# cielavenir/7bgzf

Measured on AMD Instinct MI355X. Metric: GB/s input compressed, BGZF 64KiB blocks, higher is better.
Workload: dtype u8

## Files before the change

7bgzf_amd/__init__.py:

```python
import ctypes
import os

import numpy as np

HERE = os.path.dirname(os.path.abspath(__file__))
LIB_PATH = os.path.join(HERE, "libhipdeflate.so")

FRAME_RAW, FRAME_BGZF, FRAME_MIGZ, FRAME_RAW_FLUSH, FRAME_ZLIB, FRAME_GZIP = 0, 1, 2, 3, 4, 5
FRAME_LATENCY = 0x100
DEFLATE_HIP = 11
HD_E_NODEVICE, HD_E_ARG, HD_E_NOMEM = 100, 101, 102

BGZF_BLOCK = 0xff00
WG_LEVEL = 3
BGZF_EOF = bytes.fromhex("1f8b08040000000000ff0600424302001b0003000000000000000000")


class HipDeflateError(RuntimeError):
    pass


_lib = None
_vp = ctypes.c_void_p


class MemberSummary(ctypes.Structure):
    _fields_ = [("nmembers", ctypes.c_uint64), ("out_bytes", ctypes.c_uint64), ("end_offset", ctypes.c_uint64),
                ("status", ctypes.c_uint32)]


class RangeSummary(ctypes.Structure):
    _fields_ = [("out_bytes", ctypes.c_uint64), ("nselected", ctypes.c_uint64), ("sel_bytes", ctypes.c_uint64),
                ("nrefused", ctypes.c_uint64), ("bad_member", ctypes.c_uint64), ("status", ctypes.c_uint32)]


class StreamSummary(ctypes.Structure):
    _fields_ = [("out_bytes", ctypes.c_uint64), ("in_bytes", ctypes.c_uint64), ("bad_chunk", ctypes.c_uint64),
                ("nchunks", ctypes.c_uint32), ("check", ctypes.c_uint32), ("status", ctypes.c_uint32)]


class StreamIndexSummary(ctypes.Structure):
    _fields_ = [("nchunks", ctypes.c_uint64), ("out_bytes", ctypes.c_uint64), ("end_offset", ctypes.c_uint64),
                ("ncandidates", ctypes.c_uint64), ("hdr_bytes", ctypes.c_uint32), ("status", ctypes.c_uint32)]


STREAM_WINDOW_BYTES = 1 << 30
CHECK_CRC32, CHECK_ADLER32 = 0, 1
RANGE_BYTES, RANGE_VOFFSET = 0, 1
RANGE_PIECE = 256 << 10


def voffset(coffset, uoffset):
    return (int(coffset) << 16) | (int(uoffset) & 0xffff)


EXPORTS = [
    "hipdeflate_init", "hipdeflate_shutdown", "hipdeflate_available", "hipdeflate_version", "hipdeflate_stall_count",
    "hip_deflate", "hip_deflate_flush", "hip_inflate", "hipdeflate_batch_deflate", "hipdeflate_batch_inflate",
    "hipdeflate_batch_deflate_dev", "hipdeflate_batch_inflate_dev", "hipdeflate_scan_sizes_dev",
    "hipdeflate_compact_dev", "hipdeflate_scratch_bytes", "bgzf_compress", "hipdeflate_selftest",
    "hipdeflate_pipe_open", "hipdeflate_pipe_input", "hipdeflate_pipe_submit", "hipdeflate_pipe_result",
    "hipdeflate_pipe_close", "hipdeflate_unpipe_open", "hipdeflate_unpipe_input", "hipdeflate_unpipe_submit",
    "hipdeflate_unpipe_result", "hipdeflate_unpipe_close", "hipdeflate_test_build_lengths", "hipdeflate_test_beside",
    "hip_inflate_flush", "hipdeflate_batch_inflate_flush", "hipdeflate_batch_inflate_flush_dev", "hipdeflate_bound",
    "hipdeflate_compact_span_dev", "hipdeflate_index_members_dev", "hipdeflate_verify_members_dev",
    "hipdeflate_read_ranges_dev",
    "hipdeflate_stream_bound", "hipdeflate_stream_deflate_dev", "hipdeflate_stream_inflate_dev",
    "hipdeflate_check_combine_dev", "hip_deflate_stream", "hipdeflate_test_stream_window",
    "hipdeflate_stream_index_dev", "hipdeflate_stream_inflate_table_dev", "hip_inflate_stream",
    "hipdeflate_init_devices", "hipdeflate_device_count", "hipdeflate_use_device",
    "hipdeflate_pipe_open_on", "hipdeflate_unpipe_open_on", "hipdeflate_lat_open_on",
    "hipdeflate_batch_inflate_size_dev", "hipdeflate_batch_inflate_framed_dev", "hipdeflate_batch_inflate_size",
    "hipdeflate_batch_inflate_framed",
    "hipdeflate_pipe_members", "hipdeflate_lat_open", "hipdeflate_lat_input", "hipdeflate_lat_run", "hipdeflate_lat_output", "hipdeflate_lat_close",
]


def _link_hip_runtime():
    import importlib.util
    spec = importlib.util.find_spec("torch")
    link = os.path.join(HERE, "hiprt", "libamdhip64.so.7")
    target = None
    if spec is not None and spec.submodule_search_locations:
        cand = os.path.join(list(spec.submodule_search_locations)[0], "lib", "libamdhip64.so")
        if os.path.exists(cand):
            target = cand
    try:
        if target is None:
            if os.path.islink(link) or os.path.exists(link):
                os.remove(link)
        elif not (os.path.islink(link) and os.readlink(link) == target):
            os.makedirs(os.path.dirname(link), exist_ok=True)
            if os.path.islink(link) or os.path.exists(link):
                os.remove(link)
            os.symlink(target, link)
    except OSError:
        pass


def lib():
    global _lib
    if _lib is not None:
        return _lib
    if not os.path.exists(LIB_PATH):
        raise HipDeflateError(
            "%s is missing: build it with `python -c 'import __graft_entry__ as g; g.build()'` "
            "(make -C 7bgzf_amd/csrc). There is no CPU fallback." % LIB_PATH)
    _link_hip_runtime()
    L = ctypes.CDLL(LIB_PATH)
    L.hipdeflate_version.restype = ctypes.c_char_p
    L.hipdeflate_scratch_bytes.restype = ctypes.c_uint64
    L.hipdeflate_bound.restype = ctypes.c_uint64
    L.hipdeflate_bound.argtypes = [ctypes.c_uint64, ctypes.c_int]
    L.hipdeflate_init.argtypes = [ctypes.c_int]
    L.hipdeflate_stall_count.restype = ctypes.c_uint64
    L.hipdeflate_stall_count.argtypes = []
    L.hipdeflate_init_devices.argtypes = [_vp, ctypes.c_int]
    L.hipdeflate_use_device.argtypes = [ctypes.c_int]
    L.hipdeflate_pipe_open_on.restype = _vp
    L.hipdeflate_pipe_open_on.argtypes = [ctypes.c_int, ctypes.c_int, ctypes.c_int, ctypes.c_uint32, ctypes.c_uint32, ctypes.c_int]
    L.hipdeflate_unpipe_open_on.restype = _vp
    L.hipdeflate_unpipe_open_on.argtypes = [ctypes.c_int, ctypes.c_uint32, ctypes.c_size_t, ctypes.c_size_t, ctypes.c_int]
    L.hipdeflate_lat_open_on.restype = _vp
    L.hipdeflate_lat_open_on.argtypes = [ctypes.c_int, ctypes.c_int, ctypes.c_int, ctypes.c_uint32, ctypes.c_uint32]
    sz_p = ctypes.POINTER(ctypes.c_size_t)
    L.hip_deflate.argtypes = [_vp, sz_p, _vp, ctypes.c_size_t, ctypes.c_int]
# ... 16 lines not shown
    L.hipdeflate_batch_inflate_framed.argtypes = [_vp, _vp, _vp, ctypes.c_uint32, ctypes.c_int, _vp, _vp, _vp, _vp, _vp, _vp, _vp]
    L.hipdeflate_scan_sizes_dev.argtypes = [_vp, ctypes.c_uint32, ctypes.c_uint64, _vp, _vp, _vp]
    L.hipdeflate_compact_dev.argtypes = [_vp, ctypes.c_uint64, _vp, _vp, ctypes.c_uint32, _vp, _vp]
    L.hipdeflate_compact_span_dev.argtypes = [_vp, ctypes.c_uint64, _vp, _vp, ctypes.c_uint32, _vp, ctypes.c_uint64, _vp]
    L.hipdeflate_index_members_dev.argtypes = [_vp, ctypes.c_uint64, ctypes.c_uint32, _vp, _vp, _vp, _vp, _vp,
                                               ctypes.POINTER(MemberSummary), _vp]
    L.hipdeflate_verify_members_dev.argtypes = [_vp, _vp, _vp, _vp, _vp, ctypes.c_uint32, ctypes.POINTER(ctypes.c_uint64), _vp]
    L.hipdeflate_read_ranges_dev.argtypes = [_vp, _vp, _vp, _vp, _vp, _vp, ctypes.c_uint32, ctypes.c_int, _vp, _vp, ctypes.c_uint32,
                                             _vp, ctypes.c_uint64, _vp, _vp, _vp, ctypes.POINTER(RangeSummary), _vp]
    L.hipdeflate_stream_bound.restype = ctypes.c_uint64
    L.hipdeflate_stream_bound.argtypes = [ctypes.c_uint64, ctypes.c_uint32, ctypes.c_int, ctypes.c_int]
    L.hipdeflate_stream_deflate_dev.argtypes = [_vp, ctypes.c_uint64, ctypes.c_uint32, ctypes.c_int, ctypes.c_int, _vp,
                                                ctypes.c_uint64, _vp, ctypes.POINTER(StreamSummary), _vp]
    L.hipdeflate_stream_inflate_dev.argtypes = [_vp, ctypes.c_uint64, ctypes.c_int, _vp, ctypes.c_uint32, ctypes.c_uint32,
                                                ctypes.c_uint64, _vp, ctypes.c_uint64, ctypes.POINTER(StreamSummary), _vp]
    L.hipdeflate_check_combine_dev.argtypes = [_vp, _vp, ctypes.c_uint32, ctypes.c_int, ctypes.POINTER(ctypes.c_uint32), _vp]
    L.hip_deflate_stream.argtypes = [_vp, sz_p, _vp, ctypes.c_size_t, ctypes.c_int, ctypes.c_int, ctypes.c_uint32]
    L.hipdeflate_stream_index_dev.argtypes = [_vp, ctypes.c_uint64, ctypes.c_int, ctypes.c_uint32, ctypes.c_uint32, _vp, _vp, _vp, _vp,
                                              ctypes.POINTER(StreamIndexSummary), _vp]
    L.hipdeflate_stream_inflate_table_dev.argtypes = [_vp, ctypes.c_uint64, ctypes.c_int, _vp, _vp, _vp, _vp, ctypes.c_uint32, _vp,
                                                      ctypes.c_uint64, ctypes.POINTER(StreamSummary), _vp]
    L.hip_inflate_stream.argtypes = [_vp, sz_p, _vp, ctypes.c_size_t, ctypes.c_int, sz_p]
    L.hipdeflate_test_stream_window.argtypes = [ctypes.c_uint32]
    L.hipdeflate_test_stream_window.restype = None
    L.hipdeflate_pipe_open.restype = _vp
    L.hipdeflate_pipe_open.argtypes = [ctypes.c_int, ctypes.c_int, ctypes.c_uint32, ctypes.c_uint32, ctypes.c_int]
    L.hipdeflate_pipe_input.restype = _vp
    L.hipdeflate_pipe_input.argtypes = [_vp, sz_p]
    L.hipdeflate_pipe_submit.argtypes = [_vp, ctypes.c_size_t]
    L.hipdeflate_pipe_result.argtypes = [_vp, ctypes.POINTER(_vp), sz_p, ctypes.POINTER(ctypes.c_uint32)]
    L.hipdeflate_pipe_members.argtypes = [_vp, ctypes.POINTER(_vp), ctypes.POINTER(_vp), ctypes.POINTER(_vp)]
    L.hipdeflate_pipe_close.restype = None
    L.hipdeflate_pipe_close.argtypes = [_vp]
    L.hipdeflate_unpipe_open.restype = _vp
    L.hipdeflate_unpipe_open.argtypes = [ctypes.c_uint32, ctypes.c_size_t, ctypes.c_size_t, ctypes.c_int]
    L.hipdeflate_unpipe_input.restype = _vp
    L.hipdeflate_unpipe_input.argtypes = [_vp, sz_p]
    L.hipdeflate_unpipe_submit.argtypes = [_vp, _vp, _vp, _vp, ctypes.c_uint32]
    L.hipdeflate_unpipe_result.argtypes = [_vp, ctypes.POINTER(_vp), sz_p]
    L.hipdeflate_unpipe_close.restype = None
    L.hipdeflate_unpipe_close.argtypes = [_vp]
    L.hipdeflate_lat_open.restype = _vp
    L.hipdeflate_lat_open.argtypes = [ctypes.c_int, ctypes.c_int, ctypes.c_uint32, ctypes.c_uint32]
    L.hipdeflate_lat_input.restype = _vp
    L.hipdeflate_lat_input.argtypes = [_vp, ctypes.c_uint32]
    L.hipdeflate_lat_run.argtypes = [_vp, _vp, ctypes.c_uint32]
    L.hipdeflate_lat_output.restype = _vp
    L.hipdeflate_lat_output.argtypes = [_vp, ctypes.c_uint32, _vp, _vp, _vp]
    L.hipdeflate_lat_close.restype = None
    L.hipdeflate_lat_close.argtypes = [_vp]
    L.hipdeflate_test_build_lengths.argtypes = [_vp, ctypes.c_uint32, ctypes.c_uint32, ctypes.c_uint32, _vp]
    L.hipdeflate_test_beside.argtypes = [ctypes.c_int, ctypes.c_uint32]
    L.hipdeflate_test_beside.restype = None
    _lib = L
    return L


def _check(rc, what):
    if rc:
        raise HipDeflateError("%s failed with %d%s" % (
            what, rc, " (no usable gfx950 device; there is no CPU fallback)" if rc == HD_E_NODEVICE else ""))


def available():
    return lib().hipdeflate_available() == 0


def version():
    lib().hipdeflate_available()
    return lib().hipdeflate_version().decode()


def _np(a, dtype):
    return np.ascontiguousarray(a, dtype=dtype)


def _p(a):
    return a.ctypes.data_as(_vp)


def as_u8(data):
    if isinstance(data, np.ndarray):
        return np.ascontiguousarray(data, dtype=np.uint8)
    return np.frombuffer(bytes(data), dtype=np.uint8) if len(data) else np.zeros(0, dtype=np.uint8)




def hip_deflate(data, level=1, cap=None):
    src = as_u8(data)
    cap = (len(src) + len(src) // 2 + 64) if cap is None else cap
    dst = np.zeros(max(cap, 1), dtype=np.uint8)
    n = ctypes.c_size_t(cap)
    r = lib().hip_deflate(_p(dst), ctypes.byref(n), _p(src), len(src), level)
    return r, bytes(dst[: n.value]) if r == 0 else b""


def hip_deflate_flush(data, level=1, cap=None):
    src = as_u8(data)
    cap = (len(src) + len(src) // 2 + 64) if cap is None else cap
    dst = np.zeros(max(cap, 1), dtype=np.uint8)
    n = ctypes.c_size_t(cap)
    r = lib().hip_deflate_flush(_p(dst), ctypes.byref(n), _p(src), len(src), level)
    return r, bytes(dst[: n.value]) if r == 0 else b""


# ... 258 lines not shown
```

7bgzf_amd/csrc/hd_api.hip:

```cpp
#include <hip/hip_runtime.h>
#include <stdio.h>
#include <stdlib.h>
#include <string.h>
#include <chrono>
#include <condition_variable>
#include <mutex>
#include <vector>

#include "../../include/hipdeflate.h"
#include "hd_call_batch.h"
#include "hd_deflate_static.hpp"
#include "hd_deflate_dynamic.hpp"
#include "hd_deflate_wg.hpp"
#include "hd_emit_wg.hpp"
#include "hd_inflate.hpp"
#include "hd_inflate_lat.hpp"
#include "hd_inflate_size.hpp"
#include "hd_frame.hpp"
#include "hd_compact.hpp"
#include "hd_index.hpp"
#include "hd_range.hpp"
#include "hd_stream.hpp"
#include "hd_segment.hpp"
#include "hd_tables.hpp"
// ... 54 lines not shown
			return 0;
		void *old = p;
		const size_t old_cap = cap;
		p = nullptr;
		cap = 0;
		const int r = reserve(n);
		if (r) {
			p = old;
			cap = old_cap;
			return r;
		}
		if (old)
			retired.push_back(old);
		return r;
	}
};

struct SharedScratch {
	Buf buf;
	hipEvent_t ev = nullptr;
	hipStream_t last = nullptr;
	bool used = false;
	int enter(hipStream_t st)
	{
		if (!ev)
			HD_CHECK(hipEventCreateWithFlags(&ev, hipEventDisableTiming));
		if (used && last != st)
			HD_CHECK(hipStreamWaitEvent(st, ev, 0));
		return 0;
	}
	int leave(hipStream_t st)
	{
		HD_CHECK(hipEventRecord(ev, st));
		last = st;
		used = true;
		return 0;
	}
	void drained(hipStream_t st)
	{
		if (last == st)
			used = false;
	}
	void reset()
	{
		buf.release();
		if (ev)
			(void)hipEventDestroy(ev);
		ev = nullptr;
		last = nullptr;
		used = false;
	}
};

struct Ctx {
	bool ready = false;
	int failed = 0;
	int device = -1;
	char desc[256] = "hipdeflate (not initialised)";
	hipStream_t stream = nullptr;
	CrcTables *d_ct = nullptr;
	uint32_t *d_stalls = nullptr;
	std::mutex mu;
	Buf d_in, d_meta, d_slots, d_packed, d_scratch;
	Buf h_in{ nullptr, 0, true }, h_meta{ nullptr, 0, true }, h_out{ nullptr, 0, true };
	std::mutex mu_dev;
	SharedScratch tok, tiles;
	SharedScratch frame;
	hd::WgBeside beside;
	void stream_drained(hipStream_t st)
	{
		std::lock_guard<std::mutex> lk(mu_dev);
		tok.drained(st);
		tiles.drained(st);
		frame.drained(st);
	}
	std::mutex mu_index;
	Buf d_index, d_cand;
	Buf d_range, d_range_out;
	Buf d_stream, d_stream_slots;
};

constexpr int HD_MAX_CTX = 32;
Ctx g_all[HD_MAX_CTX];
int g_want[HD_MAX_CTX];
int g_nctx = 0;
thread_local int t_cur = 0;
std::mutex g_init_mu;
inline Ctx &cur() { return g_all[t_cur]; }

}
int hd_probe_lds_order(void);
namespace {
constexpr int CODEC_LEVELS = 13;
constexpr size_t CODEC_POOL_MAX = 64;
std::mutex g_codec_mu;
std::vector<hipdeflate_lat *> g_codec_free[CODEC_LEVELS];
void codec_pool_drain()
{
	std::lock_guard<std::mutex> lk(g_codec_mu);
	for (std::vector<hipdeflate_lat *> &f : g_codec_free) {
		for (hipdeflate_lat *c : f)
			hipdeflate_lat_close(c);
		f.clear();
	}
}

void build_crc_tables(CrcTables *t)
{
	const uint32_t poly = 0xEDB88320u;
	for (uint32_t i = 0; i < 256; i++) {
		uint32_t c = i;
		for (int k = 0; k < 8; k++)
			c = (c >> 1) ^ (poly & (0u - (c & 1u)));
		t->T[0][i] = c;
	}
	for (int k = 1; k < 4; k++)
		for (uint32_t i = 0; i < 256; i++)
			t->T[k][i] = (t->T[k - 1][i] >> 8) ^ t->T[0][t->T[k - 1][i] & 0xff];
	for (int k = 0; k < 4; k++)
		for (uint32_t i = 0; i < 256; i++) {
			uint32_t s = i << (8 * k);
// ... 390 lines not shown

int hipdeflate_use_device(int index)
{
	if (index < 0 || index >= hipdeflate_device_count())
		return HD_E_ARG;
	t_cur = index;
	return ensure();
}

int hipdeflate_available(void) { return ensure(); }

uint64_t hipdeflate_stall_count(void)
{
	uint64_t sum = 0;
	std::lock_guard<std::mutex> lk(g_init_mu);
	for (int i = 0; i < HD_MAX_CTX; i++) {
		Ctx &g = g_all[i];
		if (!g.ready || !g.d_stalls)
			continue;
		uint32_t v = 0;
		if (hipSetDevice(g.device) == hipSuccess && hipDeviceSynchronize() == hipSuccess &&
		    hipMemcpy(&v, g.d_stalls, 4, hipMemcpyDeviceToHost) == hipSuccess)
			sum += v;
	}
	return sum;
}

const char *hipdeflate_version(void) { return cur().desc; }

static void infb_drain();

void hipdeflate_shutdown(void)
{
	codec_pool_drain();
	infb_drain();
	std::lock_guard<std::mutex> lk(g_init_mu);
	for (int i = 0; i < HD_MAX_CTX; i++) {
		Ctx &g = g_all[i];
		g.failed = 0;
		if (!g.ready)
			continue;
		(void)hipSetDevice(g.device);
		(void)hipDeviceSynchronize();
		for (Buf *b : { &g.d_in, &g.d_meta, &g.d_slots, &g.d_packed, &g.d_scratch, &g.h_in, &g.h_meta, &g.h_out, &g.d_index,
				&g.d_cand, &g.d_range, &g.d_range_out, &g.d_stream, &g.d_stream_slots })
			b->release();
		(void)hipFree(g.d_ct);
		(void)hipFree(g.d_stalls);
		g.d_stalls = nullptr;
		(void)hipStreamDestroy(g.stream);
		g.tok.reset();
		g.tiles.reset();
		g.frame.reset();
		g.beside.release();
		g.d_ct = nullptr;
		g.stream = nullptr;
		g.ready = false;
	}
	g_nctx = 0;
}

static uint64_t scratch_need(uint32_t nblocks, uint32_t cap, int level, bool latency)
{
	if (level >= 1 && level < HD_WG_LEVEL && latency && cap > HD_LAT_SEG_BYTES(level))
		return hd::segmented_scratch_bytes(nblocks, cap, level, HD_LAT_SEG_BYTES(level));
	if (level >= 1 && level < HD_WG_LEVEL && cap > HD_SEG_LIMIT)
		return hd::segmented_scratch_bytes(nblocks, cap, level);
	return level < 2 ? 0 : hd::dynamic_scratch_bytes(nblocks, cap, level, 0, latency);
}

uint64_t hipdeflate_scratch_bytes(uint32_t nblocks, uint32_t max_block, int level)
{
	return scratch_need(nblocks, max_block, level, false);
}

static uint64_t bound_payload(uint64_t block_bytes, int level)
{
	const uint32_t lat = HD_LAT_SEG_BYTES(level);
	return (level >= 1 && level < HD_WG_LEVEL && block_bytes > lat) ? HD_SEGN_WORST(block_bytes, lat, 0)
								: block_bytes + 5 * (block_bytes / 65535 + 1) + 5;
}

uint64_t hipdeflate_bound(uint64_t block_bytes, int level)
{
	return (bound_payload(block_bytes, level) + 32 + 15) & ~(uint64_t)15;
}


static uint32_t g_test_beside_keep = hd::BESIDE_KEEP_MAX;
static bool beside_allowed()
{
	auto on = [](const char *name) {
		const char *v = getenv(name);
		return v && *v && strcmp(v, "0") != 0;
	};
	return !on("HIPDEFLATE_NO_BESIDE") && !on("HIP_LAUNCH_BLOCKING") && !on("AMD_SERIALIZE_KERNEL") && !on("ROCPROF_COUNTER_COLLECTION") &&
	       !getenv("ROCPROF_COUNTERS");
}

struct SegRule {
	uint32_t bytes, limit;
};
static SegRule seg_rule(int level, bool latency, uint32_t room)
{
	const uint32_t seg = latency ? HD_LAT_SEG_BYTES(level) : HD_SEG_BYTES, lim = latency ? seg : HD_SEG_LIMIT;
	return { seg, (level >= 1 && level < HD_WG_LEVEL && room > lim) ? lim : 0u };
}

static hd::DeflateArgs deflate_args(const Ctx &g, const void *in, const uint64_t *in_off, const uint32_t *in_len, uint32_t nblocks,
				    int level, int frame, bool latency, void *out, uint64_t out_stride, uint32_t out_cap,
				    uint32_t *out_len, uint32_t *crc, int32_t *status, uint32_t room, uint32_t max_in)
{
	hd::DeflateArgs a{};
	a.in = (const uint8_t *)in;
	a.in_off = in_off;
	a.in_len = in_len;
	a.nblocks = nblocks;
	a.frame = frame;
	a.level = level;
	a.out = (uint8_t *)out;
	a.out_stride = out_stride;
	a.out_cap = out_cap;
	a.out_len = out_len;
	a.crc = crc;
	a.status = status;
	a.ct = g.d_ct;
	a.stalls = g.d_stalls;
	const SegRule seg = seg_rule(level, latency, room);
	a.seg_bytes = seg.bytes;
	a.seg_limit = seg.limit;
	a.split_max = (level >= HD_WG_LEVEL && max_in) ? max_in : room;
	a.lat = (latency && level >= HD_WG_LEVEL && a.split_max <= hd::EW_BLOCK_MAX) ? 1u : 0u;
	return a;
}

static int batch_deflate_dev_impl(const void *in, const void *in_off, const void *in_len, uint32_t nblocks, int level,
				  int frame, void *out, uint64_t out_stride, uint32_t out_cap, void *out_len,
				  void *crc32, void *status, void *stream, uint32_t max_in)
{
	Ctx &g = cur();
	int r = ensure();
	if (r)
		return r;
	const bool latency = (frame & HD_FRAME_LATENCY) != 0;
	frame &= ~HD_FRAME_LATENCY;
	if (frame < HD_FRAME_RAW || frame > HD_FRAME_GZIP || (out_stride & 15) || ((uintptr_t)out & 15) || !out_len)
		return HD_E_ARG;
	hipStream_t st = (hipStream_t)stream;
	hd::DeflateArgs a = deflate_args(g, in, (const uint64_t *)in_off, (const uint32_t *)in_len, nblocks, level, frame, latency, out,
					 out_stride, out_cap, (uint32_t *)out_len, (uint32_t *)crc32, (int32_t *)status,
					 hd::split_max_block(out_stride, out_cap), max_in);
	const uint64_t need = scratch_need(nblocks, a.split_max, level, latency);
	if (!need)
		return launch_deflate(a, level, st);
	std::lock_guard<std::mutex> lk(g.mu_dev);
	bool beside_fits = true;
	if (g.tok.buf.grow_keep_old(need)) {
		const uint64_t extra = (level >= HD_WG_LEVEL && !a.lat) ? hd::wg_beside_bytes(nblocks, a.split_max) : 0;
		if (!extra || extra >= need || g.tok.buf.grow_keep_old(need - extra))
			return HD_E_NOMEM;
		beside_fits = false;
	}
	a.scratch = (uint8_t *)g.tok.buf.p;
	if ((r = g.tok.enter(st)))
		return r;
	if (level >= HD_WG_LEVEL && !a.lat && beside_fits && beside_allowed() && g.beside.init() == 0) {
		a.beside = &g.beside;
		const uint32_t keep = (HD_WG_WAYS(level) == 4 && a.split_max <= 65536) ? 2u : 3u;
		a.beside_keep = g_test_beside_keep < keep ? g_test_beside_keep : keep;
	}
	if ((r = launch_deflate(a, level, st)))
		return r;
	return g.tok.leave(st);
}

int hipdeflate_batch_deflate_dev(const void *in, const void *in_off, const void *in_len, uint32_t nblocks, int level,
				 int frame, void *out, uint64_t out_stride, uint32_t out_cap, void *out_len,
				 void *crc32, void *status, void *stream)
{
	return batch_deflate_dev_impl(in, in_off, in_len, nblocks, level, frame, out, out_stride, out_cap, out_len, crc32, status,
				      stream, 0);
}

static hd::InflateArgs inflate_args(const Ctx &g, const void *in, const hd::DecTable &t, uint32_t nblocks, void *out, bool want_crc,
				    uint32_t flags)
{
	return { (const uint8_t *)in, t.in_off(), t.in_len(), nblocks, (uint8_t *)out, t.out_off(), t.out_cap(), t.out_len(),
		 want_crc ? t.crc() : nullptr, t.status(), g.d_ct, flags };
}

static int launch_inflate(const hd::InflateArgs &a, hipStream_t st)
{
	hipLaunchKernelGGL(hd::k_inflate, dim3(a.nblocks), dim3(64), 0, st, a);
	HD_CHECK(hipGetLastError());
	return 0;
}

static int batch_inflate_dev(const void *in, const void *in_off, const void *in_len, uint32_t nblocks, void *out,
			     const void *out_off, const void *out_cap, void *out_len, void *crc32, void *status, void *stream,
			     uint32_t flags)
{
	Ctx &g = cur();
	int r = ensure();
	if (r)
		return r;
	if (!out_len)
		return HD_E_ARG;
	if (nblocks == 0)
		return 0;
	return launch_inflate({ (const uint8_t *)in, (const uint64_t *)in_off, (const uint32_t *)in_len, nblocks, (uint8_t *)out,
				(const uint64_t *)out_off, (const uint32_t *)out_cap, (uint32_t *)out_len, (uint32_t *)crc32,
				(int32_t *)status, g.d_ct, flags },
			      (hipStream_t)stream);
}

int hipdeflate_batch_inflate_dev(const void *in, const void *in_off, const void *in_len, uint32_t nblocks, void *out,
				 const void *out_off, const void *out_cap, void *out_len, void *crc32, void *status,
				 void *stream)
{
	return batch_inflate_dev(in, in_off, in_len, nblocks, out, out_off, out_cap, out_len, crc32, status, stream, 0);
}

int hipdeflate_batch_inflate_flush_dev(const void *in, const void *in_off, const void *in_len, uint32_t nblocks, void *out,
				       const void *out_off, const void *out_cap, void *out_len, void *crc32, void *status,
				       void *stream)
// ... 81 lines not shown
	}
	std::lock_guard<std::mutex> lk(g.mu_dev);
	FrameTable t;
	if ((r = frame_table(g, nblocks, st, t)))
		return r;
	hipLaunchKernelGGL(hd::k_frame_open, dim3(nblocks), dim3(64), 0, st, (const uint8_t *)in, (const uint64_t *)in_off,
			   (const uint32_t *)in_len, nblocks, frame, t.p_off, t.p_len, t.verdict);
	a.in_off = t.p_off;
	a.in_len = t.p_len;
	a.crc = frame == HD_FRAME_GZIP ? t.chk : nullptr;
	hipLaunchKernelGGL(hd::k_inflate_framed, dim3(nblocks), dim3(64), 0, st, hd::InflateFramedArgs{ a, t.used });
	if (frame == HD_FRAME_ZLIB)
		hipLaunchKernelGGL(hd::k_chunk_adler, dim3(nblocks), dim3(64), 0, st, (const uint8_t *)out, (const uint64_t *)out_off,
				   (const uint32_t *)out_len, (const uint32_t *)out_cap, nblocks, t.chk);
	hipLaunchKernelGGL(hd::k_frame_close, dim3((nblocks + 255) / 256), dim3(256), 0, st, (const uint8_t *)in,
			   (const uint64_t *)in_off, (const uint64_t *)t.p_off, (const int32_t *)t.verdict, (const uint32_t *)t.used,
			   (const uint32_t *)t.chk, nblocks, frame, (uint32_t *)out_len, (uint32_t *)check, (uint32_t *)in_used,
			   (int32_t *)status);
	HD_CHECK(hipGetLastError());
	return g.frame.leave(st);
}

int hipdeflate_scan_sizes_dev(const void *out_len, uint32_t nblocks, uint64_t base, void *dst_off, void *total,
			      void *stream)
{
	Ctx &g = cur();
	int r = ensure();
	if (r)
		return r;
	if (nblocks == 0) {
		if (total)
			HD_CHECK(hipMemsetAsync(total, 0, 8, (hipStream_t)stream));
		return 0;
	}
	const uint32_t ntiles = (nblocks + hd::SCAN_TILE - 1) / hd::SCAN_TILE;
	std::lock_guard<std::mutex> lk(g.mu_dev);
	if (g.tiles.buf.grow_keep_old((size_t)ntiles * 8))
		return HD_E_NOMEM;
	uint64_t *tiles = (uint64_t *)g.tiles.buf.p;
	hipStream_t st = (hipStream_t)stream;
	if ((r = g.tiles.enter(st)))
		return r;
	hipLaunchKernelGGL(hd::k_scan_tile_sums, dim3(ntiles), dim3(256), 0, st, (const uint32_t *)out_len, nblocks, tiles);
	hipLaunchKernelGGL(hd::k_scan_tiles, dim3(1), dim3(256), 0, st, tiles, ntiles, base, (uint64_t *)total);
	hipLaunchKernelGGL(hd::k_scan_finish, dim3(ntiles), dim3(256), 0, st, (const uint32_t *)out_len, nblocks, tiles,
			   (uint64_t *)dst_off);
	HD_CHECK(hipGetLastError());
	return g.tiles.leave(st);
}

int hipdeflate_compact_dev(const void *slots, uint64_t stride, const void *out_len, const void *dst_off,
			   uint32_t nblocks, void *dst, void *stream)
{
	int r = ensure();
	if (r)
		return r;
	if (nblocks == 0)
		return 0;
	if ((stride & 3) || ((uintptr_t)slots & 3))
		return HD_E_ARG;
	hd::launch_compact((const uint8_t *)slots, stride, (const uint32_t *)out_len, (const uint64_t *)dst_off, nblocks,
			   (uint8_t *)dst, (hipStream_t)stream);
	HD_CHECK(hipGetLastError());
	return 0;
}

int hipdeflate_compact_span_dev(const void *slots, uint64_t stride, const void *out_len, const void *dst_off,
				uint32_t nblocks, void *span, uint64_t span_base, void *stream)
{
	return hipdeflate_compact_dev(slots, stride, out_len, dst_off, nblocks, (uint8_t *)span - span_base, stream);
}


static void index_scan(const uint32_t *len, uint32_t n, uint64_t *tiles, uint64_t *dst, uint64_t *total, hipStream_t st,
		       uint64_t base = 0)
{
	const uint32_t ntiles = (n + hd::SCAN_TILE - 1) / hd::SCAN_TILE;
	hipLaunchKernelGGL(hd::k_scan_tile_sums, dim3(ntiles), dim3(256), 0, st, len, n, tiles);
	hipLaunchKernelGGL(hd::k_scan_tiles, dim3(1), dim3(256), 0, st, tiles, ntiles, base, total);
	hipLaunchKernelGGL(hd::k_scan_finish, dim3(ntiles), dim3(256), 0, st, len, n, tiles, dst);
}

int hipdeflate_index_members_dev(const void *blob, uint64_t nbytes, uint32_t max_members, void *in_off, void *in_len,
				 void *out_size, void *out_off, void *crc_want, hipdeflate_member_summary *summary, void *stream)
{
	Ctx &g = cur();
	int r = ensure();
	if (r)
		return r;
	if (!summary || ((uintptr_t)blob & 15) || (nbytes && !blob))
		return HD_E_ARG;
	memset(summary, 0, sizeof *summary);
	if (nbytes == 0)
		return 0;
	hipStream_t st = (hipStream_t)stream;
	const uint8_t *src = (const uint8_t *)blob;
	std::lock_guard<std::mutex> lk(g.mu_index);
	const uint64_t nwords = (nbytes + hd::IDX_WORD - 1) / hd::IDX_WORD;
	const uint64_t ntb64 = (nwords + hd::IDX_TILE_WORDS - 1) / hd::IDX_TILE_WORDS;
	if (ntb64 > 0x7fffffffu)
		return HD_E_ARG;
	const uint32_t ntb = (uint32_t)ntb64;
	const size_t scan_tiles_a = (ntb + hd::SCAN_TILE - 1) / hd::SCAN_TILE;
	if (g.d_index.reserve(64 + (scan_tiles_a + ntb + nwords) * 8 + (size_t)ntb * 4))
		return HD_E_NOMEM;
	uint64_t *sum = (uint64_t *)g.d_index.p, *tiles_a = sum + 8, *tile_off = tiles_a + scan_tiles_a;
	uint64_t *bitmap = tile_off + ntb;
	uint32_t *tile_cnt = (uint32_t *)(bitmap + nwords);
	HD_CHECK(hipMemsetAsync(sum, 0, 64, st));
	hipLaunchKernelGGL(hd::k_index_flag, dim3(ntb), dim3(256), 0, st, src, nbytes, bitmap, tile_cnt);
	index_scan(tile_cnt, ntb, tiles_a, tile_off, sum + 4, st);
	HD_CHECK(hipGetLastError());
	uint64_t h[4] = { 0, 0, 0, 0 };
	HD_CHECK(hipMemcpyAsync(h, sum + 4, 8, hipMemcpyDeviceToHost, st));
	HD_CHECK(hipStreamSynchronize(st));
	if (h[0] > 0x7fffffffu)
// ... 1562 lines not shown
{
	hd_cb_drain(&g_infb_eng);
}

static int inflate_alone(unsigned char *dest, size_t *destLen, const unsigned char *source, size_t sourceLen, uint32_t flags)
{
	uint64_t ioff = 0, ooff = 0;
	uint32_t ilen = (uint32_t)sourceLen, olen = 0;
	uint32_t ocap = *destLen > 0xfffffff0u ? 0xfffffff0u : (uint32_t)*destLen;
	int32_t st = 0;
	int r = batch_inflate_host(source, &ioff, &ilen, 1, dest, &ooff, &ocap, &olen, nullptr, &st, flags);
	if (r)
		return r;
	if (st)
		return st;
	*destLen = olen;
	return 0;
}

static int inflate_one(unsigned char *dest, size_t *destLen, const unsigned char *source, size_t sourceLen, uint32_t flags)
{
	if (!dest || !destLen || (!source && sourceLen) || sourceLen >= HD_INFLATE_MAX_IN)
		return HD_E_ARG;
	const size_t ocap = *destLen > 0xfffffff0u ? 0xfffffff0u : *destLen;
	const size_t in_need = up16(sourceLen + 4), out_need = up16(ocap);
	if (in_need > INFB_IN_ARENA / 4 || out_need > INFB_OUT_ARENA / 4)
		return inflate_alone(dest, destLen, source, sourceLen, flags);

	const InfCall c = { sourceLen, ocap, in_need, out_need, flags };
	hd_cb_seat s;
	if (const int f = hd_cb_join(&g_infb_eng, &c, &s))
		return f == HD_E_NOMEM ? inflate_alone(dest, destLen, source, sourceLen, flags) : f;
	const InfBatch &b = g_infb[s.k];
	const hd::DecTable t = b.table();
	if (sourceLen)
		memcpy((uint8_t *)b.h_in.p + t.in_off()[s.idx], source, sourceLen);
	int ret = hd_cb_wait(&g_infb_eng, &s);
	if (!ret && !(ret = t.status()[s.idx])) {
		const uint32_t olen = t.out_len()[s.idx];
		if (olen)
			memcpy(dest, (const uint8_t *)b.h_out.p + t.out_off()[s.idx], olen);
		*destLen = olen;
	}
	hd_cb_leave(&g_infb_eng, &s);
	return ret;
}

void hipdeflate_test_beside(int keep, uint32_t sub_cap)
{
	g_test_beside_keep = keep < 0 ? 0u : (uint32_t)keep > hd::BESIDE_KEEP_MAX ? hd::BESIDE_KEEP_MAX : (uint32_t)keep;
	hd::wg_sub_test() = sub_cap;
}

#ifdef HD_EMIT_STATS
int hipdeflate_test_emit_stats(uint64_t *out16)
{
	HD_CHECK(hipDeviceSynchronize());
	HD_CHECK(hipMemcpyFromSymbol(out16, HIP_SYMBOL(hd::g_emit_stats), 128));
	return 0;
}
int hipdeflate_test_emit_stats32(uint64_t *out32)
{
	HD_CHECK(hipDeviceSynchronize());
	HD_CHECK(hipMemcpyFromSymbol(out32, HIP_SYMBOL(hd::g_emit_stats), 256));
	return 0;
}
#endif

#ifdef HD_CLOCK_STAMPS
int hipdeflate_test_clock_marks(uint64_t *out16)
{
	HD_CHECK(hipDeviceSynchronize());
	HD_CHECK(hipMemcpyFromSymbol(out16, HIP_SYMBOL(hd::g_clk_mark), 128));
	static const uint64_t zero[16] = { 0 };
	HD_CHECK(hipMemcpyToSymbol(HIP_SYMBOL(hd::g_clk_mark), zero, 128));
	return 0;
}
int hipdeflate_test_clock(uint64_t *out16)
{
	HD_CHECK(hipDeviceSynchronize());
	HD_CHECK(hipMemcpyFromSymbol(out16, HIP_SYMBOL(hd::g_clk), 128));
	static const uint64_t zero[16] = { 0 };
	HD_CHECK(hipMemcpyToSymbol(HIP_SYMBOL(hd::g_clk), zero, 128));
	return 0;
}
#endif

#ifdef HD_INFLATE_STATS
int hipdeflate_test_inflate_stats(uint64_t *out8)
{
	HD_CHECK(hipDeviceSynchronize());
	HD_CHECK(hipMemcpyFromSymbol(out8, HIP_SYMBOL(hd::g_inf_stats), 64));
	return 0;
}
int hipdeflate_test_inflate_stats2(uint64_t *out8)
{
	HD_CHECK(hipDeviceSynchronize());
	HD_CHECK(hipMemcpyFromSymbol(out8, HIP_SYMBOL(hd::g_inf_stats2), 64));
	return 0;
}
int hipdeflate_test_inflate_cycles(uint64_t *out8)
{
	HD_CHECK(hipDeviceSynchronize());
	HD_CHECK(hipMemcpyFromSymbol(out8, HIP_SYMBOL(hd::g_inf_cycles), 64));
	return 0;
}
// ... 88 lines not shown
```

7bgzf_amd/csrc/hd_compact.hpp:

```cpp
#pragma once
#include "hd_device.hpp"
#include <atomic>

namespace hd {

constexpr uint32_t SCAN_TILE = 2048;

__global__ __launch_bounds__(256) void k_scan_tile_sums(const uint32_t *len, uint32_t n, uint64_t *tile_sum)
{
	__shared__ uint64_t wsum[4];
	const uint32_t t = threadIdx.x, tile = blockIdx.x;
	uint64_t s = 0;
	for (uint32_t i = tile * SCAN_TILE + t; i < n && i < (tile + 1) * SCAN_TILE; i += 256)
		s += len[i];
	for (int o = 32; o > 0; o >>= 1) {
		s += ((uint64_t)(uint32_t)__shfl_down((int)(uint32_t)s, o, 64)) |
		     ((uint64_t)(uint32_t)__shfl_down((int)(uint32_t)(s >> 32), o, 64) << 32);
	}
	if ((t & 63) == 0)
		wsum[t >> 6] = s;
	__syncthreads();
	if (t == 0)
		tile_sum[tile] = wsum[0] + wsum[1] + wsum[2] + wsum[3];
}
// ... 51 lines not shown
	for (int k = 0; k < 8; k++) {
		v[k] = i0 + k < n ? len[i0 + k] : 0;
		s += v[k];
	}
	const uint64_t incl = wave_incl_scan64(s);
	if (lane == 63)
		wtot[w] = incl;
	__syncthreads();
	uint64_t run = tile_off[tile] + (incl - s);
	for (uint32_t k = 0; k < w; k++)
		run += wtot[k];
#pragma unroll
	for (int k = 0; k < 8; k++) {
		if (i0 + k < n)
			dst_off[i0 + k] = run;
		run += v[k];
	}
}

__device__ __forceinline__ void compact_one(const uint8_t *s, uint32_t L, uint8_t *d, uint32_t lane)
{
	uint32_t head = (uint32_t)((4 - ((uintptr_t)d & 3)) & 3);
	if (head > L)
		head = L;
	if (lane < head)
		d[lane] = s[lane];
	const uint32_t body = (L - head) >> 2;
	const uint32_t *s32 = (const uint32_t *)s;
	uint32_t *d32 = (uint32_t *)(d + head);
	for (uint32_t k = lane; k < body; k += 64) {
		const uint32_t so = head + 4 * k;
		const uint32_t lo = s32[so >> 2];
		const uint32_t hi = (so & 3) ? s32[(so >> 2) + 1] : 0;
		d32[k] = __builtin_amdgcn_alignbyte(hi, lo, so & 3);
	}
	const uint32_t done = head + 4 * body;
	if (lane < L - done)
		d[done + lane] = s[done + lane];
}

#ifndef HD_COMPACT_UNROLL
#define HD_COMPACT_UNROLL 4
#endif
#ifndef HD_COMPACT_NT
#define HD_COMPACT_NT 1
#endif
#ifndef HD_COMPACT_WAVES_PER_CU
#define HD_COMPACT_WAVES_PER_CU 3
#endif
constexpr uint32_t COMPACT_UNROLL = HD_COMPACT_UNROLL;
constexpr uint32_t COMPACT_GROUP = 64 * 16 * COMPACT_UNROLL;
constexpr bool COMPACT_NT = HD_COMPACT_NT != 0;
constexpr uint32_t COMPACT_WAVES_PER_CU = HD_COMPACT_WAVES_PER_CU;

typedef uint32_t compact_u32x4 __attribute__((ext_vector_type(4)));
typedef compact_u32x4 compact_u32x4_any __attribute__((aligned(1)));

template <bool NT>
__device__ __forceinline__ compact_u32x4 compact_ld16(const uint8_t *p)
{
	const compact_u32x4_any *q = (const compact_u32x4_any *)p;
	if (NT)
		return __builtin_nontemporal_load(q);
	return *q;
}

template <bool NT>
__device__ __forceinline__ void compact_st16(uint8_t *p, compact_u32x4 v)
{
	compact_u32x4 *q = (compact_u32x4 *)p;
	if (NT)
		__builtin_nontemporal_store(v, q);
	else
		*q = v;
}

template <bool NT, uint32_t U>
__device__ __forceinline__ void compact_wide(const uint8_t *__restrict__ s, uint32_t L, uint8_t *__restrict__ d, uint32_t lane)
{
	uint32_t head = (uint32_t)(0 - (uintptr_t)d) & 15;
	if (head > L)
		head = L;
	const uint32_t lines = (L - head) >> 4;
	const uint32_t done = head + 16 * lines;
	const uint32_t eo = lane < 16 ? lane : done + lane - 16;
	const bool edge = lane < 16 ? lane < head : lane < 32 && lane - 16 < L - done;
	uint8_t eb = 0;
	if (edge)
		eb = s[eo];
	const uint8_t *sb = s + head + 16 * lane;
	uint8_t *db = d + head + 16 * lane;
	uint32_t k = 0;
	for (; k + 64 * U <= lines; k += 64 * U) {
		compact_u32x4 v[U];
#pragma unroll
		for (uint32_t j = 0; j < U; j++)
			v[j] = compact_ld16<NT>(sb + 16 * (k + 64 * j));
#pragma unroll
		for (uint32_t j = 0; j < U; j++)
			compact_st16<NT>(db + 16 * (k + 64 * j), v[j]);
	}
	if (k < lines) {
		compact_u32x4 v[U];
		uint32_t q[U];
#pragma unroll
		for (uint32_t j = 0; j < U; j++) {
			q[j] = k + 64 * j + lane;
			v[j] = compact_ld16<NT>(s + head + 16 * (uint64_t)(q[j] < lines ? q[j] : lines - 1));
		}
#pragma unroll
		for (uint32_t j = 0; j < U; j++)
			if (q[j] < lines)
				compact_st16<NT>(d + head + 16 * (uint64_t)q[j], v[j]);
	}
	if (edge)
		d[eo] = eb;
}

__global__ __launch_bounds__(64) void k_compact(const uint8_t *__restrict__ slots, uint64_t stride, const uint32_t *__restrict__ len,
						const uint64_t *__restrict__ dst_off, uint32_t n, uint8_t *__restrict__ dst)
{
	const uint32_t lane = threadIdx.x, step = gridDim.x;
	uint32_t i = blockIdx.x;
	if (i >= n)
		return;
	uint32_t L = len[i];
	uint64_t o = dst_off[i];
	for (;;) {
		const uint32_t nx = i + step;
		const bool more = nx < n && nx > i;
		const uint32_t nc = more ? nx : i;
		const uint32_t Ln = len[nc];
		const uint64_t on = dst_off[nc];
		compact_wide<COMPACT_NT, COMPACT_UNROLL>(slots + (uint64_t)i * stride, L, dst + o, lane);
		if (!more)
			break;
		i = nx;
		L = Ln;
		o = on;
	}
}

inline uint32_t compact_device_cus()
{
	static std::atomic<uint32_t> cus[64];
	int dev = 0;
	if (hipGetDevice(&dev) != hipSuccess || dev < 0 || dev >= 64)
		return 256;
	uint32_t c = cus[dev].load(std::memory_order_relaxed);
	if (!c) {
		int v = 0;
		if (hipDeviceGetAttribute(&v, hipDeviceAttributeMultiprocessorCount, dev) != hipSuccess || v <= 0)
			v = 256;
		cus[dev].store(c = (uint32_t)v, std::memory_order_relaxed);
	}
	return c;
}

inline void launch_compact(const uint8_t *slots, uint64_t stride, const uint32_t *len, const uint64_t *dst_off, uint32_t n,
			   uint8_t *dst, hipStream_t st)
{
	const uint64_t cap = (uint64_t)compact_device_cus() * COMPACT_WAVES_PER_CU;
	hipLaunchKernelGGL(k_compact, dim3(n < cap ? n : (uint32_t)cap), dim3(64), 0, st, slots, stride, len, dst_off, n, dst);
}

__global__ __launch_bounds__(64) void k_adler32_patch(const uint8_t *in, const uint64_t *in_off, const uint32_t *in_len,
						      uint32_t nblocks, uint8_t *out, uint64_t out_stride,
						      const uint32_t *out_len, const int32_t *status)
{
	const uint32_t b = blockIdx.x, lane = threadIdx.x;
	if (b >= nblocks || (status && status[b]) || out_len[b] < 6)
		return;
	const uint8_t *src = in + in_off[b];
	const uint32_t n = in_len[b];
	const bool aligned = (((uintptr_t)src) & 15) == 0;
	AdlerLanes adl;
	adl.init();
	for (uint32_t piece = 0; piece * HD_PIECE < n; piece++) {
		const uint32_t o = piece * HD_PIECE + lane * 16;
		uint4 v = make_uint4(0, 0, 0, 0);
		if (aligned && o + 16 <= n) {
			v = *(const uint4 *)(src + o);
		} else if (o < n) {
			uint32_t w[4] = { 0, 0, 0, 0 };
#pragma unroll
			for (uint32_t k = 0; k < 16; k++)
				w[k >> 2] |= (o + k < n ? (uint32_t)src[o + k] : 0u) << (8 * (k & 3));
			v = make_uint4(w[0], w[1], w[2], w[3]);
		}
		adl.fold(piece, lane, v);
	}
	const uint32_t a = adl.finish(n);
	if (lane < 4)
		out[(uint64_t)b * out_stride + out_len[b] - 4 + lane] = (uint8_t)(a >> (24 - 8 * lane));
}

}
```

include/hipdeflate.h:

```cpp
#ifndef HIPDEFLATE_H
#define HIPDEFLATE_H

#include <stddef.h>
#include <stdint.h>

#ifdef __cplusplus
extern "C" {
#endif

#define DEFLATE_HIP 11

#define HD_E_NODEVICE  100
#define HD_E_ARG       101
#define HD_E_NOMEM     102

#define HD_FRAME_RAW   0
#define HD_FRAME_BGZF  1
#define HD_FRAME_MIGZ  2
#define HD_FRAME_RAW_FLUSH 3
#define HD_FRAME_ZLIB  4
#define HD_FRAME_GZIP  5

#define HD_FRAME_LATENCY 0x100

// ... 140 lines not shown
int hipdeflate_stream_index_dev(const void *strm, uint64_t nbytes, int frame, uint32_t max_chunks, uint32_t max_chunk_in,
				void *in_off , void *in_len , void *out_size , void *out_off ,
				hipdeflate_stream_index_summary *summary , void *stream);
int hipdeflate_stream_inflate_table_dev(const void *strm, uint64_t nbytes, int frame,
					const void *in_off, const void *in_len, const void *out_size, const void *out_off,
					uint32_t nchunks, void *out, uint64_t out_cap,
					hipdeflate_stream_summary *summary , void *stream);
int hip_inflate_stream(unsigned char *dest, size_t *destLen, const unsigned char *source, size_t sourceLen, int frame,
		       size_t *in_used);
int hipdeflate_check_combine_dev(const void *check, const void *len, uint32_t n, int kind, uint32_t *result, void *stream);
int hip_deflate_stream(unsigned char *dest, size_t *destLen, const unsigned char *source, size_t sourceLen,
		       int level, int frame, uint32_t chunk_bytes);
void hipdeflate_test_stream_window(uint32_t chunks);

typedef struct hipdeflate_pipe hipdeflate_pipe;
hipdeflate_pipe *hipdeflate_pipe_open(int level, int frame, uint32_t block_bytes,
				      uint32_t blocks_per_batch, int depth);
uint8_t *hipdeflate_pipe_input(hipdeflate_pipe *p, size_t *cap);
int hipdeflate_pipe_submit(hipdeflate_pipe *p, size_t nbytes);
int hipdeflate_pipe_result(hipdeflate_pipe *p, const uint8_t **data, size_t *nbytes,
			   uint32_t *nblocks);
int hipdeflate_pipe_members(hipdeflate_pipe *p, const uint32_t **out_len, const uint64_t **dst_off,
			    const uint32_t **crc32);
#define HIPDEFLATE_VOFFSET(coffset, uoffset) (((uint64_t)(coffset) << 16) | (uint64_t)((uoffset) & 0xffff))
void hipdeflate_pipe_close(hipdeflate_pipe *p);
hipdeflate_pipe *hipdeflate_pipe_open_on(int index, int level, int frame, uint32_t block_bytes,
					 uint32_t blocks_per_batch, int depth);

typedef struct hipdeflate_unpipe hipdeflate_unpipe;
hipdeflate_unpipe *hipdeflate_unpipe_open(uint32_t max_members, size_t in_cap, size_t out_cap, int depth);
uint8_t *hipdeflate_unpipe_input(hipdeflate_unpipe *p, size_t *cap);
int hipdeflate_unpipe_submit(hipdeflate_unpipe *p, const uint64_t *in_off, const uint32_t *in_len,
			     const uint32_t *out_size, uint32_t nmembers);
int hipdeflate_unpipe_result(hipdeflate_unpipe *p, const uint8_t **data, size_t *nbytes);
void hipdeflate_unpipe_close(hipdeflate_unpipe *p);
hipdeflate_unpipe *hipdeflate_unpipe_open_on(int index, uint32_t max_members, size_t in_cap, size_t out_cap, int depth);

typedef struct hipdeflate_lat hipdeflate_lat;
hipdeflate_lat *hipdeflate_lat_open(int level, int frame, uint32_t max_blocks, uint32_t max_block_bytes);
uint8_t *hipdeflate_lat_input(hipdeflate_lat *c, uint32_t i);
int hipdeflate_lat_run(hipdeflate_lat *c, const uint32_t *in_len, uint32_t n);
const uint8_t *hipdeflate_lat_output(hipdeflate_lat *c, uint32_t i, uint32_t *out_len, uint32_t *crc32, int32_t *status);
void hipdeflate_lat_close(hipdeflate_lat *c);
hipdeflate_lat *hipdeflate_lat_open_on(int index, int level, int frame, uint32_t max_blocks, uint32_t max_block_bytes);

uint64_t hipdeflate_scratch_bytes(uint32_t nblocks, uint32_t max_block, int level);

int bgzf_compress(void *dst, size_t *dlen, const void *src, size_t slen, int level);

int hipdeflate_selftest(void);
int hipdeflate_test_build_lengths(const uint32_t *freq, uint32_t nvec, uint32_t nsyms, uint32_t maxbits,
				  uint8_t *lens_out);
void hipdeflate_test_beside(int keep, uint32_t sub_cap);

#ifdef __cplusplus
}
#endif
#endif
```

Before: 385.0.

## Shrink compact grid when a large encode is still running on another stream

Records an event after each deflate launch. When a compact is issued on a different stream while a large level≥1 encode is still in flight, the compact kernel is launched with a small grid (about half a wave per CU) so it runs beside the encode instead of competing with it for CUs. An env var can force either grid. This adds an event record and query per call, and the small grid could slow the compact when overlap does not actually happen.

```diff
diff --git a/7bgzf_amd/__init__.py b/7bgzf_amd/__init__.py
--- a/7bgzf_amd/__init__.py
+++ b/7bgzf_amd/__init__.py
@@ -72,6 +72,7 @@
     "hipdeflate_pipe_open_on", "hipdeflate_unpipe_open_on", "hipdeflate_lat_open_on",
     "hipdeflate_batch_inflate_size_dev", "hipdeflate_batch_inflate_framed_dev", "hipdeflate_batch_inflate_size",
     "hipdeflate_batch_inflate_framed",
+    "hipdeflate_test_compact_grid",
     "hipdeflate_pipe_members", "hipdeflate_lat_open", "hipdeflate_lat_input", "hipdeflate_lat_run", "hipdeflate_lat_output", "hipdeflate_lat_close",
 ]
 
@@ -194,6 +195,8 @@
     L.hipdeflate_test_build_lengths.argtypes = [_vp, ctypes.c_uint32, ctypes.c_uint32, ctypes.c_uint32, _vp]
     L.hipdeflate_test_beside.argtypes = [ctypes.c_int, ctypes.c_uint32]
     L.hipdeflate_test_beside.restype = None
+    L.hipdeflate_test_compact_grid.argtypes = []
+    L.hipdeflate_test_compact_grid.restype = ctypes.c_uint32
     _lib = L
     return L
 
diff --git a/7bgzf_amd/csrc/hd_api.hip b/7bgzf_amd/csrc/hd_api.hip
--- a/7bgzf_amd/csrc/hd_api.hip
+++ b/7bgzf_amd/csrc/hd_api.hip
@@ -130,6 +130,22 @@
 	}
 };
 
+struct LastEncode {
+	hipEvent_t ev = nullptr;
+	hipStream_t stream = nullptr;
+	const void *out = nullptr;
+	int level = 0;
+	uint32_t nblocks = 0;
+	bool valid = false;
+	void reset()
+	{
+		if (ev)
+			(void)hipEventDestroy(ev);
+		ev = nullptr;
+		valid = false;
+	}
+};
+
 struct Ctx {
 	bool ready = false;
 	int failed = 0;
@@ -145,6 +161,9 @@
 	SharedScratch tok, tiles;
 	SharedScratch frame;
 	hd::WgBeside beside;
+	std::mutex mu_enc;
+	LastEncode enc;
+	uint32_t compact_grid = 0;
 	void stream_drained(hipStream_t st)
 	{
 		std::lock_guard<std::mutex> lk(mu_dev);
@@ -641,6 +660,7 @@
 		g.tok.reset();
 		g.tiles.reset();
 		g.frame.reset();
+		g.enc.reset();
 		g.beside.release();
 		g.d_ct = nullptr;
 		g.stream = nullptr;
@@ -685,6 +705,60 @@
 	};
 	return !on("HIPDEFLATE_NO_BESIDE") && !on("HIP_LAUNCH_BLOCKING") && !on("AMD_SERIALIZE_KERNEL") && !on("ROCPROF_COUNTER_COLLECTION") &&
 	       !getenv("ROCPROF_COUNTERS");
+}
+
+constexpr uint32_t ENCODE_L1_WAVES_PER_CU = 21;
+static bool stream_capturing(hipStream_t st)
+{
+	hipStreamCaptureStatus s = hipStreamCaptureStatusNone;
+	if (hipStreamIsCapturing(st, &s) != hipSuccess) {
+		(void)hipGetLastError();
+		return true;
+	}
+	return s != hipStreamCaptureStatusNone;
+}
+
+static void note_encode(Ctx &g, hipStream_t st, const void *out, int level, uint32_t nblocks)
+{
+	if (!nblocks || stream_capturing(st))
+		return;
+	std::lock_guard<std::mutex> lk(g.mu_enc);
+	LastEncode &e = g.enc;
+	e.valid = false;
+	if (!e.ev && hipEventCreateWithFlags(&e.ev, hipEventDisableTiming) != hipSuccess) {
+		e.ev = nullptr;
+		(void)hipGetLastError();
+		return;
+	}
+	if (hipEventRecord(e.ev, st) != hipSuccess) {
+		(void)hipGetLastError();
+		return;
+	}
+	e.stream = st;
+	e.out = out;
+	e.level = level;
+	e.nblocks = nblocks;
+	e.valid = true;
+}
+
+static bool compact_beside(Ctx &g, const void *slots, hipStream_t st)
+{
+	const char *v = getenv("HIPDEFLATE_GATHER_GRID");
+	if (v && !strcmp(v, "full"))
+		return false;
+	if (v && !strcmp(v, "beside"))
+		return true;
+	if (stream_capturing(st))
+		return false;
+	std::lock_guard<std::mutex> lk(g.mu_enc);
+	const LastEncode &e = g.enc;
+	if (!e.valid || e.stream == st || e.out == slots || e.level < 1 ||
+	    e.nblocks < (uint64_t)hd::compact_device_cus() * ENCODE_L1_WAVES_PER_CU)
+		return false;
+	const hipError_t q = hipEventQuery(e.ev);
+	if (q != hipSuccess)
+		(void)hipGetLastError();
+	return q == hipErrorNotReady;
 }
 
 struct SegRule {
@@ -740,8 +814,12 @@
 					 out_stride, out_cap, (uint32_t *)out_len, (uint32_t *)crc32, (int32_t *)status,
 					 hd::split_max_block(out_stride, out_cap), max_in);
 	const uint64_t need = scratch_need(nblocks, a.split_max, level, latency);
-	if (!need)
-		return launch_deflate(a, level, st);
+	if (!need) {
+		if ((r = launch_deflate(a, level, st)))
+			return r;
+		note_encode(g, st, out, level, nblocks);
+		return 0;
+	}
 	std::lock_guard<std::mutex> lk(g.mu_dev);
 	bool beside_fits = true;
 	if (g.tok.buf.grow_keep_old(need)) {
@@ -760,6 +838,7 @@
 	}
 	if ((r = launch_deflate(a, level, st)))
 		return r;
+	note_encode(g, st, out, level, nblocks);
 	return g.tok.leave(st);
 }
 
@@ -947,6 +1026,7 @@
 int hipdeflate_compact_dev(const void *slots, uint64_t stride, const void *out_len, const void *dst_off,
 			   uint32_t nblocks, void *dst, void *stream)
 {
+	Ctx &g = cur();
 	int r = ensure();
 	if (r)
 		return r;
@@ -954,9 +1034,12 @@
 		return 0;
 	if ((stride & 3) || ((uintptr_t)slots & 3))
 		return HD_E_ARG;
-	hd::launch_compact((const uint8_t *)slots, stride, (const uint32_t *)out_len, (const uint64_t *)dst_off, nblocks,
-			   (uint8_t *)dst, (hipStream_t)stream);
+	hipStream_t st = (hipStream_t)stream;
+	const uint32_t grid = hd::launch_compact((const uint8_t *)slots, stride, (const uint32_t *)out_len, (const uint64_t *)dst_off,
+						 nblocks, (uint8_t *)dst, st, compact_beside(g, slots, st));
 	HD_CHECK(hipGetLastError());
+	std::lock_guard<std::mutex> lk(g.mu_enc);
+	g.compact_grid = grid;
 	return 0;
 }
 
@@ -2625,6 +2708,13 @@
 	hd::wg_sub_test() = sub_cap;
 }
 
+uint32_t hipdeflate_test_compact_grid(void)
+{
+	Ctx &g = cur();
+	std::lock_guard<std::mutex> lk(g.mu_enc);
+	return g.compact_grid;
+}
+
 #ifdef HD_EMIT_STATS
 int hipdeflate_test_emit_stats(uint64_t *out16)
 {
diff --git a/7bgzf_amd/csrc/hd_compact.hpp b/7bgzf_amd/csrc/hd_compact.hpp
--- a/7bgzf_amd/csrc/hd_compact.hpp
+++ b/7bgzf_amd/csrc/hd_compact.hpp
@@ -127,6 +127,11 @@
 constexpr uint32_t COMPACT_GROUP = 64 * 16 * COMPACT_UNROLL;
 constexpr bool COMPACT_NT = HD_COMPACT_NT != 0;
 constexpr uint32_t COMPACT_WAVES_PER_CU = HD_COMPACT_WAVES_PER_CU;
+#ifndef HD_COMPACT_BESIDE_WAVES_PER_2CU
+#define HD_COMPACT_BESIDE_WAVES_PER_2CU 1
+#endif
+constexpr uint32_t COMPACT_BESIDE_WAVES_PER_2CU = HD_COMPACT_BESIDE_WAVES_PER_2CU;
+static_assert(COMPACT_BESIDE_WAVES_PER_2CU >= 1 && COMPACT_BESIDE_WAVES_PER_2CU <= 2 * COMPACT_WAVES_PER_CU, "the small grid is not above the full one");
 
 typedef uint32_t compact_u32x4 __attribute__((ext_vector_type(4)));
 typedef compact_u32x4 compact_u32x4_any __attribute__((aligned(1)));
@@ -232,11 +237,16 @@
 	return c;
 }
 
-inline void launch_compact(const uint8_t *slots, uint64_t stride, const uint32_t *len, const uint64_t *dst_off, uint32_t n,
-			   uint8_t *dst, hipStream_t st)
-{
-	const uint64_t cap = (uint64_t)compact_device_cus() * COMPACT_WAVES_PER_CU;
-	hipLaunchKernelGGL(k_compact, dim3(n < cap ? n : (uint32_t)cap), dim3(64), 0, st, slots, stride, len, dst_off, n, dst);
+inline uint32_t launch_compact(const uint8_t *slots, uint64_t stride, const uint32_t *len, const uint64_t *dst_off, uint32_t n,
+			       uint8_t *dst, hipStream_t st, bool beside = false)
+{
+	const uint64_t cus = compact_device_cus();
+	uint64_t cap = beside ? cus * COMPACT_BESIDE_WAVES_PER_2CU / 2 : cus * COMPACT_WAVES_PER_CU;
+	if (!cap)
+		cap = 1;
+	const uint32_t grid = n < cap ? n : (uint32_t)cap;
+	hipLaunchKernelGGL(k_compact, dim3(grid), dim3(64), 0, st, slots, stride, len, dst_off, n, dst);
+	return grid;
 }
 
 __global__ __launch_bounds__(64) void k_adler32_patch(const uint8_t *in, const uint64_t *in_off, const uint32_t *in_len,
diff --git a/include/hipdeflate.h b/include/hipdeflate.h
--- a/include/hipdeflate.h
+++ b/include/hipdeflate.h
@@ -216,6 +216,7 @@
 int hipdeflate_test_build_lengths(const uint32_t *freq, uint32_t nvec, uint32_t nsyms, uint32_t maxbits,
 				  uint8_t *lens_out);
 void hipdeflate_test_beside(int keep, uint32_t sub_cap);
+uint32_t hipdeflate_test_compact_grid(void);
 
 #ifdef __cplusplus
 }
```

Result: faster. 392.5, median of 6 (+1.9%).
